# fengpeng-yue/speech-to-speech-translation

Measured on AMD Instinct MI355X. Metric: mel-frames/sec (fwd+bwd+opt) on Fisher-shaped fbank80->mel80, higher is better.
Workload: dtype bf16; 1 GPU; s2st_transformer base 12enc/6dec d512 nfps4 + aux ASR/ST(1x64) + CTC, recipe dropouts, max-tokens=20000 Fisher-shaped batches, update-freq 1; parallelism=dp1

## Files before the change

include/s2st_hip.h:

```cpp
#ifndef S2ST_HIP_H
#define S2ST_HIP_H
#include <stdint.h>
#ifdef __cplusplus
extern "C" {
#endif

#define S2ST_OK 0
#define S2ST_ERR_LAUNCH (-1)
#define S2ST_ERR_SHAPE (-2)
#define S2ST_ERR_WORKSPACE (-3)
#define S2ST_ERR_ARG (-4)
#define S2ST_ERR_COMM (-5)

typedef struct { int64_t ld; int64_t bs; int32_t per; int32_t _pad; } s2st_split;

typedef struct {
  const void* p;
  int32_t kmajor;
  int32_t dtype;
  s2st_split sp;
  int64_t zo, zi;
} s2st_gemm_operand;

#define S2ST_F32 0
// ... 212 lines not shown
int s2st_engine_create(const s2st_model_config* cfg, s2st_engine** out);
void s2st_engine_destroy(s2st_engine* e);
int32_t s2st_engine_num_params(const s2st_engine* e);
int s2st_engine_param_info(const s2st_engine* e, int32_t i, s2st_param_info* out);
int64_t s2st_engine_param_floats(const s2st_engine* e);
int64_t s2st_engine_buffer_floats(const s2st_engine* e);
int s2st_engine_bind(s2st_engine* e, float* params, float* grads, float* buffers);
int s2st_engine_bind_bf16(s2st_engine* e, uint16_t* params_bf16);
int s2st_engine_bf16_is_fresh(s2st_engine* e);
int64_t s2st_engine_stall_report(s2st_engine* e, int32_t verbose);
#define S2ST_SITE_LINEAR 1
#define S2ST_SITE_ATTN 2
#define S2ST_SITE_ROWS 3
#define S2ST_SITE_NORM 4
typedef struct s2st_dropout_site {
  uint64_t seed;
  int32_t kind;
  int32_t ordinal;
  float p;
  int32_t reserved;
  int64_t dims[5];
  char ctx[24];
} s2st_dropout_site;
int s2st_engine_allow_side_stream(s2st_engine* e, int32_t allow);
int s2st_engine_site_log(s2st_engine* e, int32_t on);
int32_t s2st_engine_site_log_get(const s2st_engine* e, s2st_dropout_site* out, int32_t cap);
int s2st_engine_bind_bf16_transposed(s2st_engine* e, uint16_t* params_bf16_t);
int64_t s2st_engine_workspace_floats(s2st_engine* e, const s2st_batch* geometry);
int s2st_engine_forward(s2st_engine* e, const s2st_batch* b, const s2st_outputs* out,
                        float* workspace, int64_t workspace_floats, void* stream);
int s2st_engine_backward(s2st_engine* e, float gscale, int32_t segment, void* stream);
int32_t s2st_engine_num_segments(const s2st_engine* e);
void* s2st_engine_side_stream(const s2st_engine* e);
int s2st_engine_segment_range(const s2st_engine* e, int32_t i, int64_t* lo, int64_t* hi);
int s2st_engine_adam_overlapped(s2st_engine* e, float* exp_avg, float* exp_avg_sq, const float* sumsq_parts, int32_t n_parts, float gmul, const float* gmul_dev, float max_norm, float lr, float beta1, float beta2, float eps, float wd, int32_t step, float* gnorm_out, int32_t* skipped, int32_t write_bf16, int32_t n_chunks, void* stream);
int s2st_engine_wait_optimizer(s2st_engine* e, void* stream);

int64_t s2st_engine_decode_state_floats(const s2st_engine* e, int32_t B, int32_t E, int32_t max_steps);
int s2st_engine_decode_begin(s2st_engine* e, const s2st_batch* b, const s2st_outputs* out, float* state,
                             int64_t state_floats, int32_t max_steps, float* workspace,
                             int64_t workspace_floats, void* stream);
int s2st_engine_decode_row_map(s2st_engine* e, const int32_t* row_map);
int s2st_engine_decode_step(s2st_engine* e, int32_t step, const float* prev, const int32_t* pos,
                            const int32_t* self_klen ,
                            uint64_t seed, float* feat_out, float* eos_prob, float* attn_out, float* workspace,
                            int64_t workspace_floats, void* stream);

typedef struct {
  int32_t* step;
  uint64_t* seeds;
  float* cur_feat;
  float* cur_eos;
  float* cur_attn;
  float* pe_cur;
} s2st_decode_replay;
int32_t s2st_engine_decode_replay_supported(const s2st_engine* e);
int s2st_engine_decode_replay_begin(s2st_engine* e, const s2st_decode_replay* r, uint64_t seed0, void* stream);
int s2st_engine_decode_step_replay(s2st_engine* e, const s2st_decode_replay* r, const int32_t* self_klen, float* workspace,
                                   int64_t workspace_floats, void* stream);
int s2st_engine_decode_replay_commit(s2st_engine* e, const s2st_decode_replay* r, uint64_t seed0, float thr, int32_t max_iter,
                                     int32_t* finished, int32_t* out_lens, int32_t* klen_next, int32_t* n_done,
                                     float* feat_all, float* eos_all, float* attn_all, void* stream);
int s2st_engine_postnet_eval(s2st_engine* e, const float* feat, int32_t B, int32_t D, float* post_out,
                             float* workspace, int64_t workspace_floats, void* stream);

int s2st_argmax_dim1_f32(const float* x, int64_t* idx, int32_t B, int32_t E, int32_t D, void* stream);
// ... 105 lines not shown
```

speech-to-speech-translation_amd/csrc/engine.cpp:

```cpp
#include <cmath>
#include <cstdio>
#include <cstdlib>
#include <cstring>
#include <functional>
#include <string>
#include <vector>

#include "s2st_ops.h"
#include <hip/hip_ext.h>

namespace {

struct PInfo {
  std::string name;
  long off, numel;
  int ndim;
  int shape[4];
  int is_buffer;
};

struct Ten {
  float* d = nullptr;
  float* g = nullptr;
  bf16raw* h = nullptr;
// ... 17 lines not shown
struct LinP { long w, b; int N, K; };
struct LNP { long g, b; int C; };
struct AttnP { long kvq_w, kvq_b, out_w, out_b; };
struct XAttnP { long kv_w, kv_b, q_w, q_b, out_w, out_b; };
struct EncLayerP { AttnP sa; LNP ln1; LinP fc1, fc2; LNP ln2; };
struct DecLayerP { AttnP sa; LNP ln1; XAttnP xa; LNP ln2; LinP fc1, fc2; LNP ln3; };
struct ConvP { long w, b; int O, I, Kw; };
struct BNP { long g, b, rm, rv; int C; };
struct AuxP {
  long embed; int V, in_dim, d, layers, out_dim;
  long proj_in;
  std::vector<DecLayerP> L;
  LNP ln; bool has_ln;
  long proj_out;
  long out_proj;
};

}

struct s2st_engine {
  s2st_model_config c;
  std::vector<PInfo> infos;
  long n_params = 0, n_buffers = 0;
  float *P = nullptr, *G = nullptr, *BUF = nullptr;
  hipStream_t side_ = nullptr;
  hipEvent_t ev_fork_ = nullptr, ev_join_ = nullptr, ev_taps_ = nullptr;
  bool overlap_aux = true;
  bool hoist_kv = true;
  hipEvent_t ev_kv_ = nullptr;
  bool kv_wait_ = false;
  hipEvent_t ev_auxb_ = nullptr;
  size_t aux_wait_idx = 0, aux_lo_idx = 0, aux_hi_idx = 0;
  bool aux_bwd_on_side = false;
  bool side_used = false;
  float* skws_side = nullptr;
  bool side_allowed = false;
  bool side_tried = false;
  void ensure_side() {
    if (side_ || side_tried || !side_allowed) return;
    side_tried = true;
    int pr_least = 0, pr_greatest = 0;
    if (hipDeviceGetStreamPriorityRange(&pr_least, &pr_greatest) != hipSuccess) pr_least = 0;
    if (hipStreamCreateWithPriority(&side_, hipStreamNonBlocking, pr_least) != hipSuccess) side_ = nullptr;
    if (side_ && hipEventCreateWithFlags(&ev_kv_, hipEventDisableTiming) != hipSuccess) ev_kv_ = nullptr;
    if (side_ && (hipEventCreateWithFlags(&ev_fork_, hipEventDisableTiming) != hipSuccess ||
                  hipEventCreateWithFlags(&ev_join_, hipEventDisableTiming) != hipSuccess ||
                  hipEventCreateWithFlags(&ev_taps_, hipEventDisableTiming) != hipSuccess ||
                  hipEventCreateWithFlags(&ev_auxb_, hipEventDisableTiming) != hipSuccess)) {
      hipStreamDestroy(side_);
      side_ = nullptr;
    }
  }
  hipStream_t fork_side() {
    if (!side_) { sync_chains(); return st_; }
    hipEventRecord(ev_fork_, st_);
    hipStreamWaitEvent(side_, ev_fork_, 0);
    if (forked_) {
      hipEventRecord(ev_cside_, chain1_);
      hipStreamWaitEvent(side_, ev_cside_, 0);
    }
    side_used = true;
    return side_;
  }
  struct Stall { const char* what; hipEvent_t a, b; };
  std::vector<Stall> stalls;
  bool stall_trace = false;
  void wait_traced(hipStream_t st, hipEvent_t ev, const char* what) {
    if (!stall_trace) { hipStreamWaitEvent(st, ev, 0); return; }
    Stall s{what, nullptr, nullptr};
    hipEventCreate(&s.a);
    hipEventCreate(&s.b);
    hipEventRecord(s.a, st);
    hipStreamWaitEvent(st, ev, 0);
    hipEventRecord(s.b, st);
    stalls.push_back(s);
  }
  void join_side() {
    sync_chains();
    if (!side_ || !side_used) return;
    hipEventRecord(ev_join_, side_);
    wait_traced(st_, ev_join_, "join_side");
    side_used = false;
  }

// ... 211 lines not shown
  e->use_skinny = !(s2st_env_on("S2ST_NO_SKINNY"));
  e->use_ln_fuse = !(s2st_env_on("S2ST_NO_LN_FUSE"));
  e->attn_gfuse_mode = s2st_env_int("S2ST_ATTN_GFUSE", 1);
  e->use_attn_gfuse = e->attn_gfuse_mode != 0;
  e->ln_bwd_split = s2st_env_on("S2ST_LN_BWD_SPLIT");
  e->ordered_sums = !(s2st_env_int("S2ST_ORDERED_BIAS_SUMS", 1) == 0);
  e->build_params();
  (void)hipGetLastError();
  if (!cfg->precise && (s2st_gemm_bf16_preload(nullptr) != 0 || s2st_flash_attn_preload(nullptr) != 0)) { delete e; return S2ST_ERR_LAUNCH; }
  e->side_allowed = !cfg->precise && !(s2st_env_on("S2ST_NO_SIDE_STREAM"));
  e->overlap_aux = !(s2st_env_on("S2ST_NO_AUX_OVERLAP"));
  if (!cfg->precise && s2st_env_int("S2ST_CHAINS", 1) == 2) {
    if (hipStreamCreateWithFlags(&e->chain1_, hipStreamNonBlocking) == hipSuccess &&
        hipEventCreateWithFlags(&e->ev_cfork_, hipEventDisableTiming) == hipSuccess &&
        hipEventCreateWithFlags(&e->ev_cjoin_, hipEventDisableTiming) == hipSuccess &&
        hipEventCreateWithFlags(&e->ev_cside_, hipEventDisableTiming) == hipSuccess)
      e->nchains = 2;
    else { delete e; return S2ST_ERR_LAUNCH; }
  }
  *out = e;
  return 0;
}

void s2st_engine_destroy(s2st_engine* e) {
  if (!e) return;
  if (e->side_) {
    hipStreamSynchronize(e->side_);
    hipStreamDestroy(e->side_);
    hipEventDestroy(e->ev_fork_);
    hipEventDestroy(e->ev_join_);
    if (e->ev_taps_) hipEventDestroy(e->ev_taps_);
    if (e->ev_auxb_) hipEventDestroy(e->ev_auxb_);
    if (e->ev_kv_) hipEventDestroy(e->ev_kv_);
    for (hipEvent_t ev : e->adam_ev) hipEventDestroy(ev);
  }
  if (e->chain1_) {
    hipStreamSynchronize(e->chain1_);
    hipStreamDestroy(e->chain1_);
    if (e->ev_cfork_) hipEventDestroy(e->ev_cfork_);
    if (e->ev_cjoin_) hipEventDestroy(e->ev_cjoin_);
    if (e->ev_cside_) hipEventDestroy(e->ev_cside_);
  }
  e->reset_call();
  delete e;
}

int32_t s2st_engine_num_params(const s2st_engine* e) { return (int32_t)e->infos.size(); }

int s2st_engine_param_info(const s2st_engine* e, int32_t i, s2st_param_info* out) {
  if (i < 0 || i >= (int)e->infos.size()) return S2ST_ERR_ARG;
  const PInfo& p = e->infos[i];
  memset(out, 0, sizeof(*out));
  strncpy(out->name, p.name.c_str(), sizeof(out->name) - 1);
  out->offset = p.off;
  out->numel = p.numel;
  out->ndim = p.ndim;
  for (int k = 0; k < 4; ++k) out->shape[k] = p.shape[k];
  out->is_buffer = p.is_buffer;
  return 0;
}

int64_t s2st_engine_param_floats(const s2st_engine* e) { return e->n_params; }
int64_t s2st_engine_buffer_floats(const s2st_engine* e) { return e->n_buffers; }

int s2st_engine_bind(s2st_engine* e, float* params, float* grads, float* buffers) {
  e->P = params;
// ... 78 lines not shown
}

int s2st_engine_backward(s2st_engine* e, float gscale, int32_t segment, void* stream) {
  if (!e->G) return S2ST_ERR_ARG;
  e->st_ = (hipStream_t)stream;
  e->gscale = gscale;
  if (segment < 0) {
    for (int s = 0; s < e->n_segments(); ++s) {
      int rc = e->backward_segment(s);
      if (rc) return rc;
    }
    return 0;
  }
  return e->backward_segment(segment);
}

int s2st_engine_adam_overlapped(s2st_engine* e, float* exp_avg, float* exp_avg_sq, const float* sumsq_parts, int32_t n_parts,
                                float gmul, const float* gmul_dev, float max_norm, float lr, float beta1, float beta2, float eps,
                                float wd, int32_t step, float* gnorm_out, int32_t* skipped, int32_t write_bf16, int32_t n_chunks,
                                void* stream) {
  if (!e || !exp_avg || !exp_avg_sq || !sumsq_parts || n_parts <= 0) return S2ST_ERR_ARG;
  return e->adam_overlapped(exp_avg, exp_avg_sq, sumsq_parts, n_parts, gmul, gmul_dev, max_norm, lr, beta1, beta2, eps, wd, step,
                            gnorm_out, skipped, write_bf16, n_chunks, (hipStream_t)stream);
}

int s2st_engine_wait_optimizer(s2st_engine* e, void* stream) {
  if (!e) return S2ST_ERR_ARG;
  e->adam_wait_all((hipStream_t)stream);
  return 0;
}

int32_t s2st_engine_num_segments(const s2st_engine* e) { return e->n_segments(); }

void* s2st_engine_side_stream(const s2st_engine* e) {
  const_cast<s2st_engine*>(e)->ensure_side();
  return (void*)e->side_;
}

int s2st_engine_segment_range(const s2st_engine* e, int32_t i, int64_t* lo, int64_t* hi) {
  int ns = e->n_segments();
  if (i < 0 || i >= ns) return S2ST_ERR_ARG;
  *lo = e->marks[ns - i - 1].param_off;
  *hi = e->marks[ns - i].param_off;
  return 0;
}

int64_t s2st_engine_decode_state_floats(const s2st_engine* e, int32_t B, int32_t E, int32_t max_steps) {
  const long Cd = e->c.dec_dim, L = e->c.dec_layers;
  return L * 2 * B * (long)max_steps * Cd + L * (long)B * E * 2 * Cd + 64 + ((long)max_steps + 2) * Cd + L * (long)B * E * Cd + 8;
}

int s2st_engine_decode_begin(s2st_engine* e, const s2st_batch* b, const s2st_outputs* out, float* state,
                             int64_t state_floats, int32_t max_steps, float* workspace, int64_t workspace_floats,
                             void* stream) {
  if (!e->P || !e->BUF || !state || !b || !out) return S2ST_ERR_ARG;
  if (state_floats < s2st_engine_decode_state_floats(e, b->B, b->E, max_steps)) return S2ST_ERR_WORKSPACE;
  e->dec_row_map = nullptr;
  e->begin_call(workspace, workspace_floats, stream);
  e->bt = *b;
  e->bt.training = 0;
  e->bt.tgt = nullptr;
  e->outs = *out;
  e->stop_after_encoder = true;
  int rc = e->forward();
  e->stop_after_encoder = false;
  if (rc) return rc;
  e->dec_st.base = state;
  e->dec_st.B = b->B; e->dec_st.E = b->E; e->dec_st.maxT = max_steps;
  e->dec_st.enc_lens = b->enc_lens;
  e->dec_st.pe_dec = b->pe_dec;
  {
    const long Cd = e->c.dec_dim, L = e->c.dec_layers;
    e->dec_st.pe_alpha = state + L * 2 * b->B * (long)max_steps * Cd + L * (long)b->B * b->E * 2 * Cd + 64;
    e->touch(e->pos_alpha + 1);
    if (e->live())
      e->chk(s2st_scale_rows(b->pe_dec, e->P + e->pos_alpha, e->dec_st.pe_alpha, ((long)max_steps + 2) * Cd, e->st_));
  }
  for (int l = 0; l < e->c.dec_layers; ++l) {
    const XAttnP& xa = e->dec[l].xa;
    e->linear(e->enc_out_keep, xa.kv_w, xa.kv_b, 2 * e->c.dec_dim, e->c.enc_dim, 0, 0.f, nullptr, e->dec_crossKV(l));
  }
  return e->end_call(0);
}

int s2st_engine_decode_row_map(s2st_engine* e, const int32_t* row_map) {
  if (!e) return S2ST_ERR_ARG;
  e->dec_row_map = row_map;
  return S2ST_OK;
}

int s2st_engine_decode_step(s2st_engine* e, int32_t step, const float* prev, const int32_t* pos,
                            const int32_t* self_klen, uint64_t seed, float* feat_out, float* eos_prob,
                            float* attn_out, float* workspace, int64_t workspace_floats, void* stream) {
  if (!e->P || !prev || !pos || !feat_out || !eos_prob) return S2ST_ERR_ARG;
  e->begin_call(workspace, workspace_floats, stream);
  if (int rc = e->params_ready(false, false)) return rc;
// ... 217 lines not shown
```

speech-to-speech-translation_amd/csrc/engine_ops.h:

```cpp
  Ten* linear(Ten* x, long w, long b, int N, int K, int act = 0, float drop_p = 0.f,
              Ten* resid = nullptr, float* ext_out = nullptr, bool only_h = false, const float* resid_row = nullptr) {
    const int M = x->rows;
    const bool fm = fast();
    const bool skinny = fm && !bt.training && use_skinny && M <= S2ST_SKINNY_MAX_ROWS && K % 32 == 0 && x->d && x->cols == K &&
                        (act == 0 || act == 1 || act == 3);
    only_h = only_h && fast() && use_only_h && N % 8 == 0 && !ext_out && !resid && !skinny;
    Ten* y = newT(M, N, ext_out, !only_h);
    touch(w + (long)N * K);
    if (b >= 0) touch(b + N);
    const uint64_t sd = drop_p > 0.f ? next_seed(S2ST_SITE_LINEAR, drop_p, M, N) : 0;
    if (skinny) {
      const uint64_t* seed_ptr = nullptr;
      if (replay_ && drop_p > 0.f) {
        if (site < 1 || site > 8) { if (!err) err = S2ST_ERR_SHAPE; return y; }
        seed_ptr = replay_->seeds + (site - 1);
      }
      if (live())
        chk(s2st_gemm_skinny(x->d, K, PH + w, K, y->d, N, b >= 0 ? P + b : nullptr, act, drop_p, sd,
                             resid ? resid->d : resid_row, resid ? N : 0, M, N, K, st_, nullptr, nullptr, 1e-5f, seed_ptr,
                             drop_p > 0.f ? dec_row_map : nullptr));
      return y;
    }
    if (replay_ && drop_p > 0.f && !err) err = S2ST_ERR_SHAPE;
    const bf16raw* xh = fm ? half_of(x) : nullptr;
// ... 380 lines not shown
      bool aq, ak, av;
      float* gq = gradbuf(io2.qt, aq);
      float* gk = gradbuf(io2.kt, ak);
      float* gv = gradbuf(io2.vt, av);
      (void)aq; (void)ak; (void)av;
      float* dp = alloc((long)B * H * T * ld);
      bf16raw* dsh = fm ? alloc_h((long)B * H * T * ld) : nullptr;
      const bf16raw* doh = fm ? ghalf_of(o) : nullptr;
      if (!live()) return;
      const View Vdo{o->g, doh};
      bgemm(Vdo, 1, C, (long)T * C, Vv, 1, io2.ldv, (long)S * io2.ldv, dp, ld, pzo, pzi, dh, dh, T, S, dh, 1.f);
      bgemm(View{pd, pdh}, 0, ld, pzo, Vdo, 0, C, (long)T * C, gv + io2.voff, io2.ldv, (long)S * io2.ldv, dh, pzi,
            dh, S, dh, T, 1.f);
      chk(s2st_softmax_bwd(p, dp, dp, B, H, T, S, ld, drop_p, sd, st_, dsh));
      bgemm(View{dp, dsh}, 1, ld, pzo, Vk, 0, io2.ldk, (long)S * io2.ldk, gq + io2.qoff, io2.ldq,
            (long)T * io2.ldq, dh, pzi, dh, T, dh, S, scaling);
      bgemm(View{dp, dsh}, 0, ld, pzo, Vq, 0, io2.ldq, (long)T * io2.ldq, gk + io2.koff, io2.ldk,
            (long)S * io2.ldk, dh, pzi, dh, S, dh, T, scaling);
    });
    return o;
  }

  Ten* self_attn_block(Ten* x, const AttnP& a, int B, int T, int H, const int* klen, int causal,
                       Ten* resid) {
    const int C = x->cols;
    Ten* kvq = linear(x, a.kvq_w, a.kvq_b, 3 * C, C, 0, 0.f, nullptr, nullptr, true);
    AttnIO io{kvq, 2 * C, 3 * C, kvq, 0, 3 * C, kvq, C, 3 * C};
    Ten* o = attention(io, B, T, T, H, C / H, klen, causal, bt.training ? c.attn_dropout : 0.f, nullptr);
    return linear(o, a.out_w, a.out_b, C, C, 0, bt.training ? c.dropout : 0.f, resid);
  }
  Ten* cross_kv(Ten* encx, const XAttnP& a, int C) {
    return linear(encx, a.kv_w, a.kv_b, 2 * C, encx->cols, 0, 0.f, nullptr, nullptr, true);
  }
  Ten* cross_attn_block(Ten* x, Ten* encx, const XAttnP& a, int B, int T, int S, int H,
                        const int* klen, Ten* resid, float* attn_mean_out, Ten* kv_pre = nullptr) {
    const int C = x->cols;
    Ten* q = linear(x, a.q_w, a.q_b, C, C, 0, 0.f, nullptr, nullptr, true);
    Ten* kv = kv_pre ? kv_pre : cross_kv(encx, a, C);
    if (kv_pre && kv_wait_) {
      wait_traced(st_, ev_kv_, "cross-attention K|V projections");
      chains_wait(ev_kv_);
      kv_wait_ = false;
    }
    AttnIO io{q, 0, C, kv, 0, 2 * C, kv, C, 2 * C};
    Ten* o = attention(io, B, T, S, H, C / H, klen, 0, bt.training ? c.attn_dropout : 0.f, attn_mean_out);
    return linear(o, a.out_w, a.out_b, C, C, 0, bt.training ? c.dropout : 0.f, resid);
  }
  Ten* ffn_block(Ten* x, const LinP& fc1, const LinP& fc2, Ten* resid) {
    Ten* h = linear(x, fc1.w, fc1.b, fc1.N, fc1.K, ffn_act, bt.training ? c.act_dropout : 0.f, nullptr, nullptr,
                    ffn_act == 1 || is_hubert);
    return linear(h, fc2.w, fc2.b, fc2.N, fc2.K, 0, bt.training ? c.dropout : 0.f, resid);
  }
  Ten* enc_layer(Ten* x, const EncLayerP& l, int B, int T) {
    const int H = c.enc_heads;
    if (c.enc_pre_ln) {
      x = self_attn_block(layernorm(x, l.ln1, nullptr, true), l.sa, B, T, H, bt.enc_lens, 0, x);
      return ffn_block(layernorm(x, l.ln2, nullptr, true), l.fc1, l.fc2, x);
    }
    x = layernorm(self_attn_block(x, l.sa, B, T, H, bt.enc_lens, 0, x), l.ln1);
    return layernorm(ffn_block(x, l.fc1, l.fc2, x), l.ln2);
  }
  Ten* dec_layer(Ten* x, Ten* encx, const DecLayerP& l, int B, int T, int S, int H, bool pre_ln,
                 const int* self_klen, float* attn_mean_out, Ten* kv_pre = nullptr) {
    if (pre_ln) {
      x = self_attn_block(layernorm(x, l.ln1, nullptr, true), l.sa, B, T, H, self_klen, 1, x);
      x = cross_attn_block(layernorm(x, l.ln2, nullptr, true), encx, l.xa, B, T, S, H, bt.enc_lens, x, attn_mean_out, kv_pre);
      return ffn_block(layernorm(x, l.ln3, nullptr, true), l.fc1, l.fc2, x);
    }
    x = layernorm(self_attn_block(x, l.sa, B, T, H, self_klen, 1, x), l.ln1);
    x = layernorm(cross_attn_block(x, encx, l.xa, B, T, S, H, bt.enc_lens, x, attn_mean_out, kv_pre), l.ln2);
    return layernorm(ffn_block(x, l.fc1, l.fc2, x), l.ln3);
  }

  struct ConvIn { float* xh; Ten* src; int Tin; const bf16raw* xhh; };
  struct ConvW { float *wf, *wd, *dwf; const bf16raw *wfh, *wdh; };
  Ten* conv(const ConvIn& in, const ConvP& p, int B, int stride, const ConvW& cw) {
    float *wf = cw.wf, *wd = cw.wd, *dwf = cw.dwf;
    const bf16raw *wfh = cw.wfh, *wdh = cw.wdh;
    const bool fm = fast();
    const int pad = p.Kw / 2;
    const int Tin = in.Tin, Tout = (Tin + 2 * pad - p.Kw) / stride + 1;
    const int Th = Tin + 2 * pad;
    Ten* z = newT(B * Tout, p.O);
    touch(p.w + (long)p.O * p.I * p.Kw);
    touch(p.b + p.O);
    if (live()) {
      GemmArgs g{};
      g.A = fm ? gemm_rowmajor(in.xhh, (long)stride * p.I) : gemm_rowmajor(in.xh, (long)stride * p.I);
      g.A.sp.per = Tout; g.A.sp.bs = (long)Th * p.I;
      g.B = fm ? gemm_rowmajor(wfh, (long)p.Kw * p.I) : gemm_rowmajor(wf, (long)p.Kw * p.I);
      g.C = gemm_out(z->d, p.O);
      g.ep = gemm_epi_default();
      g.ep.bias = P + p.b;
      g.M = B * Tout; g.N = p.O; g.K = p.Kw * p.I; g.batch = 1; g.zdiv = 1; g.precise = c.precise;
      chk(s2st_gemm(g, st_));
    }
    ConvP pp = p;
    ConvIn in2 = in;
    tape.push_back([=]() {
      if (!z->g) return;
      const int M = B * Tout;
      const bf16raw* dzh = fm ? ghalf_of(z) : nullptr;
      float* cpart = ordered_sums ? alloc(s2st_colsum_scratch_floats(M, pp.O)) : nullptr;
// ... 132 lines not shown
```

speech-to-speech-translation_amd/csrc/engine_step.h:

```cpp
  bool use_streamk = s2st_env_on("S2ST_GEMM_STREAMK");
  void reset_call() {
    pending_wgrad.clear();
    pending_lnfold = s2st_lnfold_table{};
    s2st_gemm_streamk_unbind_all();
    for (Ten* t : tens) delete t;
    tens.clear();
    tape.clear();
    tape_aware.clear();
    forked_ = false;
    in_region_ = false;
    marks.clear();
    ws_top = 0;
    ws_peak = 0;
    oom = false;
    err = 0;
    site = 0;
    site_log.clear();
    site_ctx[0] = 0;
    param_watermark = 0;
    next_segment = 0;
    skws = nullptr; skws_n = 0; skws_side = nullptr;
  }
  void begin_call(float* workspace, long workspace_floats, void* stream) {
    reset_call();
    dry = false;
    ws = workspace;
    ws_cap = workspace_floats;
    st_ = (hipStream_t)stream;
  }
  int params_ready(bool chunked = false, bool refresh = true) {
    if (dry) return 0;
    const bool fm = fast();
    if (fm && !PH) return S2ST_ERR_ARG;
    if (adam_pending && !(chunked && fm && ph_fresh)) adam_wait_all(st_);
    if (fm && refresh) {
      if (!ph_fresh) chk(s2st_cast_bf16_rows(P, n_params, PH, n_params, 1, (int)n_params, st_));
      ph_fresh = false;
    }
    return err;
  }
  int end_call(int rc) {
    tape.clear();
    return rc ? rc : err;
  }

  int forward() {
    const int B = bt.B, S = bt.S, D = bt.D, C = c.enc_dim, Cd = c.dec_dim;
    const int pad = c.conv_k / 2;
    const int T1 = c.text_input ? S : (S + 2 * pad - c.conv_k) / 2 + 1;
    const int T2 = c.text_input ? S : (T1 + 2 * pad - c.conv_k) / 2 + 1;
    if (T2 != bt.E) return S2ST_ERR_SHAPE;
    if (c.text_input && (!bt.src_txt || bt.Ls != S)) return S2ST_ERR_ARG;
    const int E = T2;
    const bool tr = bt.training != 0;
    const bool with_loss = bt.tgt != nullptr;
    seed = bt.seed;
    if (tr) ensure_side();
    main_ = st_;
    forked_ = false;
    in_region_ = false;
    const bool two_chains = nchains == 2 && chain1_ && tr && fast();

    const float *pe_enc = bt.pe_enc, *pe_dec = bt.pe_dec, *pe_asr = bt.pe_asr, *pe_st = bt.pe_st;
    const bool fm = fast();
    if (int rc = params_ready(true)) return rc;
    pht_valid = false;
    if (fm && tr && PHT && live()) {
      hipStream_t ts = side_ ? fork_side() : st_;
      if (wt_tables.empty()) build_wt_tables();
      for (const s2st_transpose_table& tb : wt_tables) chk(s2st_transpose_bf16_batched(PH, PHT, tb, ts));
      pht_valid = true;
    }
    skws_n = fm ? (long)16 << 20 : 0;
    skws = fm ? alloc(skws_n) : nullptr;
    skws_side = fm && side_allowed ? alloc(skws_n) : skws;
    skws_c1 = fm && chain1_ && nchains == 2 ? alloc(skws_n) : skws;
    if (fm && tr && use_streamk) {
      float* sk0 = alloc(S2ST_STREAMK_SCRATCH_FLOATS);
      float* sk1 = side_allowed ? alloc(S2ST_STREAMK_SCRATCH_FLOATS) : nullptr;
      if (live()) {
        hipMemsetAsync(sk0, 0, 4096, st_);
        s2st_gemm_streamk_bind(st_, sk0, S2ST_STREAMK_SCRATCH_FLOATS);
        if (sk1 && side_) {
          hipMemsetAsync(sk1, 0, 4096, st_);
          s2st_gemm_streamk_bind(side_, sk1, S2ST_STREAMK_SCRATCH_FLOATS);
        }
      }
    }
    typedef ConvW ConvScratch;
    auto conv_scratch = [&](const ConvP& p, bool need_wd) { return make_conv_scratch(p, need_wd, tr); };
    ConvScratch cs0{}, cs1{};
    std::vector<ConvScratch> cst;
    if (c.text_input) {
      for (auto& pc : enc_conv) cst.push_back(conv_scratch(pc, true));
    } else {
      cs0 = conv_scratch(sub[0], false);
      cs1 = conv_scratch(sub[1], true);
    }
    std::vector<ConvScratch> csp;
    {
      const bool post_on_side = fm && side_ && ev_taps_ && ev_kv_ && live() && hoist_kv && !stop_after_encoder &&
                                c.dec_layers > 0;
      hipStream_t main_st = st_;
      if (post_on_side) st_ = fork_side();
      for (auto& pc : post_conv) csp.push_back(conv_scratch(pc, true));
      st_ = main_st;
    }

    mark();
    Ten* x = nullptr;
    if (c.text_input) {
      Ten* emb = newT(B * E, C);
      touch(enc_embed + (long)c.src_vocab * C);
      if (live()) chk(s2st_embed_fwd((const long*)bt.src_txt, P + enc_embed, emb->d, B * E, C, 1.f, st_));
      const long eoff = enc_embed;
      tape.push_back([=]() {
        if (!emb->g) return;
        if (live()) chk(s2st_embed_bwd((const long*)bt.src_txt, emb->g, G + eoff, B * E, C, 1.f, 1, st_, ordered_sums ? c.src_vocab : 0));
      });
      set_ctx("enc.prenet");
      Ten* pn = text_prenet(emb, B, E, tr, cst);
      Ten* pj = linear(pn, enc_prenet_proj.w, enc_prenet_proj.b, C, C);
      set_ctx("enc.pe");
      x = add_pe(pj, bt.enc_pos, pe_enc, 1.f, enc_pos_alpha, tr ? c.dropout : 0.f);
    } else {
    float* xh0 = fm ? nullptr : alloc((long)B * (S + 2 * pad) * c.in_dim, true);
    if (live() && !fm) {
      Split xs{(long)c.in_dim, 0, 0, 0};
      Split ys{(long)c.in_dim, (long)(S + 2 * pad) * c.in_dim, S, 0};
      chk(s2st_copy_rows(bt.src, xs, xh0 + (long)pad * c.in_dim, ys, B * S, c.in_dim, st_));
    }
    const bf16raw* xh0h = fm ? cast_halo(bt.src, B, S, pad, c.in_dim, true) : nullptr;
    Ten* z1 = conv(ConvIn{xh0, nullptr, S, xh0h}, sub[0], B, 2, cs0);
    const int C1 = c.conv_channels / 2;
    float* g1h = alloc((long)B * (T1 + 2 * pad) * C1, !fm);
    Ten* g1 = glu_to(z1, g1h + (long)pad * C1, Split{(long)C1, (long)(T1 + 2 * pad) * C1, T1, 0}, C1);
    const bf16raw* g1hh = fm ? cast_halo(g1h, B, T1, pad, C1) : nullptr;
    Ten* z2 = conv(ConvIn{g1h, g1, T1, g1hh}, sub[1], B, 2, cs1);
// ... 32 lines not shown
        if (!c.spk_frozen && live())
          chk(s2st_speaker_cols_bwd(cat->g, (const long*)bt.speaker, B, E, C + Sd, C, Sd, c.n_speakers, G + soff, st_));
        if (xin->needs_grad) {
          bool acc;
          float* dx = gradbuf(xin, acc);
          if (live()) chk(s2st_split_cols(cat->g, C + Sd, dx, C, B * E, C, acc ? 1 : 0, st_));
        }
      });
      enc_out = linear(cat, enc_spk_proj.w, enc_spk_proj.b, C, C + Sd, 0, 0.f, nullptr, outs.enc_out);
    } else if (!has_enc_ln && outs.enc_out && live())
      hipMemcpyAsync(outs.enc_out, x->d, sizeof(float) * (size_t)x->n(), hipMemcpyDeviceToDevice, st_);
    if (!c.has_asr && tap_asr && outs.tap0 && live())
      hipMemcpyAsync(outs.tap0, tap_asr->d, sizeof(float) * (size_t)tap_asr->n(), hipMemcpyDeviceToDevice, st_);
    if (c.has_asr && tap_asr) tap_asr = layernorm(tap_asr, asr_norm, outs.tap0);
    if (c.has_st && tap_st) tap_st = layernorm(tap_st, st_norm, outs.tap1);
    const bool aux_on_side = side_ && ev_taps_ && live() && overlap_aux && !(c.text_input && c.has_ctc);
    const bool kv_on_side = side_ && ev_taps_ && ev_kv_ && live() && hoist_kv && !stop_after_encoder;
    if (aux_on_side || kv_on_side) hipEventRecord(ev_taps_, st_);
    aux_wait_idx = tape.size();
    mark();
    if (stop_after_encoder) {
      enc_out_keep = enc_out;
      return err;
    }
    if (c.s2t_mode) return forward_s2t(enc_out, with_loss);
    std::vector<Ten*> xkv(c.dec_layers, nullptr);
    if (hoist_kv) {
      hipStream_t main_st = st_;
      if (kv_on_side) {
        hipStreamWaitEvent(side_, ev_taps_, 0);
        st_ = side_;
        side_used = true;
      }
      for (int i = 0; i < c.dec_layers; ++i) xkv[i] = cross_kv(enc_out, dec[i].xa, Cd);
      if (kv_on_side) {
        hipEventRecord(ev_kv_, side_);
        st_ = main_st;
        kv_wait_ = true;
      }
      mark();
    }
    Ten* prev = newT(B * D, c.out_dim, const_cast<float*>(bt.prev));
    prev->needs_grad = false;
    if (dec_spk >= 0 && bt.speaker) {
      Ten* pv = newT(B * D, c.out_dim);
      touch_spk(dec_spk + (long)c.n_speakers * c.out_dim);
      if (live()) {
        hipMemcpyAsync(pv->d, bt.prev, sizeof(float) * (size_t)pv->n(), hipMemcpyDeviceToDevice, st_);
        chk(s2st_speaker_set_rows(spk_tab(dec_spk), (const long*)bt.speaker, pv->d, B, D, c.out_dim, st_));
      }
      pv->needs_grad = tr && !c.spk_frozen;
      const long doff = dec_spk;
      tape.push_back([=]() {
        if (!pv->g || c.spk_frozen) return;
        if (live())
          chk(s2st_speaker_bwd(pv->g, (const long*)bt.speaker, B, D, 1, c.out_dim, c.n_speakers, 0.f, 0, G + doff, st_));
      });
      prev = pv;
    }
    Ten* h = prev;
    set_ctx("dec.prenet");
    for (int i = 0; i < c.prenet_layers; ++i)
      h = linear(h, prenet[i].w, prenet[i].b, prenet[i].N, prenet[i].K, 1, c.prenet_dropout);
    h = linear(h, prenet.back().w, prenet.back().b, Cd, c.prenet_dim);
    set_ctx("dec.pe");
    Ten* y = add_pe(h, bt.dec_pos, pe_dec, 1.f, pos_alpha, tr ? c.dropout : 0.f);
    mark();
    in_region_ = two_chains;
    float* attn_out = nullptr;
    Ten* tap_dec_t = nullptr;
    for (int i = 0; i < c.dec_layers; ++i) {
      float* am = (i == c.dec_layers - 1 && bt.want_attn) ? outs.attn : nullptr;
      set_ctx("dec.L%d", i);
      y = dec_layer(y, enc_out, dec[i], B, D, E, c.dec_heads, c.dec_pre_ln != 0, bt.tgt_lens, am, xkv[i]);
      if (c.has_ctc_tgt && i == c.tap_dec) tap_dec_t = y;
      if (i % 2 == 1) mark();
    }
    (void)attn_out;
    if (has_dec_ln) y = layernorm(y, dec_ln);
    Ten* feat = linear(y, feat_proj.w, feat_proj.b, c.out_dim, Cd, 0, 0.f, nullptr, outs.feat);
    Ten* eos = linear(y, eos_proj.w, eos_proj.b, 1, Cd, 0, 0.f, nullptr, outs.eos);
    in_region_ = false;
    if (live()) sync_chains();
    set_ctx("post");
    Ten* post = postnet(feat, B, D, tr, csp, outs.post_feat);
    set_ctx("");
    Ten* ctc_tgt_logits = nullptr;
    float *ctc_tgt_per = nullptr, *ctc_tgt_dl = nullptr;
    if (c.has_ctc_tgt && tap_dec_t) {
      ctc_tgt_logits = linear(tap_dec_t, ctc_proj_tgt.w, ctc_proj_tgt.b, c.tgt_vocab, Cd);
      if (with_loss) {
        ctc_tgt_per = alloc(B);
        float* lp = alloc((long)B * D * c.tgt_vocab);
        float* wsd = alloc(s2st_ctc_workspace_floats(B, D, bt.Lt));
        ctc_tgt_dl = tr ? alloc(ctc_tgt_logits->n()) : nullptr;
        if (live())
          chk(s2st_ctc(ctc_tgt_logits->d, (const long*)bt.tgt_txt, bt.Lt, bt.tgt_lens, bt.tgt_txt_lens, B, D, c.tgt_vocab,
                       lp, ctc_tgt_per, ctc_tgt_dl, ctc_tgt_dl ? c.ctc_tgt_weight / B : 0.f, wsd, st_));
      }
    }
    mark();
    hipStream_t main_st = st_;
    aux_lo_idx = tape.size();
    if (aux_on_side) {
      hipStreamWaitEvent(side_, ev_taps_, 0);
      st_ = side_;
      side_used = true;
    }
    Ten* ctc_logits = nullptr;
    if (c.has_ctc && tap_asr && !c.text_input) ctc_logits = linear(tap_asr, ctc_proj.w, ctc_proj.b, c.src_vocab, C);
    const bool t2s_ctc = c.text_input && c.has_ctc;
// ... 113 lines not shown
        chk(s2st_loss_finalize(stats, nullptr, B, 1.f, 1.f, 0.f, 0.f, 0.f, 0.f, 1.f, 0.f, c.label_smoothing, c.tgt_vocab,
                               c.tgt_vocab, 1.f, 1.f, st_, nullptr, 0.f, ordered_sums ? &lp : nullptr));
      }
      tape.push_back([=]() {
        bool a;
        float* dl = gradbuf(logits, a);
        if (live())
          chk(s2st_ls_ce(logits->d, (const long*)bt.src_txt, B * bt.Ls, c.tgt_vocab, 1, c.label_smoothing, nullptr, dl,
                         gscale, st_));
      });
    }
    if (adam_pending && live()) adam_wait_all(st_);
    join_side();
    mark();
    return err;
  }

  int n_segments() const { return marks.empty() ? 0 : (int)marks.size() - 1; }

  int backward_segment(int seg) {
    int ns = n_segments();
    if (seg < 0 || seg >= ns) return S2ST_ERR_ARG;
    if (seg == 0) join_side();
    size_t hi = marks[ns - seg].tape_idx, lo = marks[ns - seg - 1].tape_idx;
    hipStream_t main_st = st_;
    main_ = st_;
    in_region_ = false;
    for (size_t i = hi; i-- > lo;) {
      if (aux_bwd_on_side && live()) {
        if (i + 1 == aux_hi_idx && st_ == main_st) { flush_wgrad(); flush_lnfold(); st_ = fork_side(); }
        if (i + 1 == aux_lo_idx && st_ != main_st) { flush_wgrad(); flush_lnfold(); hipEventRecord(ev_auxb_, st_); st_ = main_st; }
        if (i + 1 == aux_wait_idx) wait_traced(main_st, ev_auxb_, "aux decoders' backward (tap gradients)");
      }
      if (live() && !(i < tape_aware.size() && tape_aware[i])) sync_chains();
      tape[i]();
      if (err) break;
    }
    flush_wgrad();
    flush_lnfold();
    if (st_ != main_st) { hipEventRecord(ev_auxb_, st_); st_ = main_st; }
    if (live()) sync_chains();
    if (seg == ns - 1) join_side();
    return err;
  }
```

speech-to-speech-translation_amd/runtime/engine.py:

```python
from __future__ import annotations

import ctypes as C
import math
import os
from typing import Callable, Dict, List, Optional, Tuple

import torch

from . import binding as bd

PAD = 1


class ModelConfig(C.Structure):
    _fields_ = [(n, C.c_int32) for n in (
        "enc_layers", "dec_layers", "enc_dim", "dec_dim", "enc_ffn", "dec_ffn", "enc_heads",
        "dec_heads", "enc_pre_ln", "dec_pre_ln", "in_dim", "conv_channels", "conv_k", "out_dim",
        "prenet_layers", "prenet_dim", "postnet_layers", "postnet_dim", "postnet_k", "tap_asr",
        "tap_st", "has_asr", "has_st", "has_ctc", "asr_layers", "asr_dim", "st_layers", "st_dim",
        "src_vocab", "tgt_vocab", "no_scale_embedding", "precise", "tap_dec", "has_ctc_tgt", "text_input", "enc_conv_layers", "enc_conv_k",
        "n_speakers", "spk_frozen", "spk_dim")] + [(n, C.c_float) for n in (
        "dropout", "attn_dropout", "act_dropout", "prenet_dropout", "postnet_dropout", "ctc_weight",
        "asr_weight", "st_weight", "w_l1", "w_mse", "w_eos", "bce_pos_weight", "label_smoothing", "ctc_tgt_weight", "enc_dropout")] + \
        [("s2t_mode", C.c_int32)]
# ... 650 lines not shown
    def site_log(self, on: bool = True):
        bd.check(self.lib.s2st_engine_site_log(self.h, 1 if on else 0), "s2st_engine_site_log")

    def dropout_sites(self) -> Dict[str, "DropoutSite"]:
        f = self.lib.s2st_engine_site_log_get
        n = int(f(self.h, None, 0))
        recs = (DropoutSite * max(n, 1))()
        f(self.h, C.cast(recs, C.c_void_p), n)
        out = {}
        for r in recs[:n]:
            name = f"{r.ctx.decode()}/{SITE_KIND[r.kind]}{r.ordinal}"
            assert name not in out, name
            out[name] = r
        return out

    def dropout_keep_mask(self, site: "DropoutSite") -> torch.Tensor:
        d = [int(v) for v in site.dims]
        shape = (d[0], d[1], d[2], d[4]) if site.kind == 2 else (d[0], d[1])
        n = 1
        for v in shape:
            n *= v
        ones = torch.ones(n, dtype=torch.float32, device=self.device)
        y = torch.empty_like(ones)
        bd.call("s2st_dropout_f32", ones, y, n, 1.0, float(site.p), int(site.seed), 0)
        keep = (y != 0).float()
        return keep.view(*shape)

    def side_stream(self):
        if bd.is_emulator() or not torch.cuda.is_available():
            return None
        p = self.lib.s2st_engine_side_stream(self.h)
        return torch.cuda.ExternalStream(p) if p else None

    def num_segments(self) -> int:
        return int(self.lib.s2st_engine_num_segments(self.h))

    def segment_range(self, i: int) -> Tuple[int, int]:
        lo, hi = C.c_int64(), C.c_int64()
        bd.check(self.lib.s2st_engine_segment_range(self.h, i, C.byref(lo), C.byref(hi)), "segment_range")
        return int(lo.value), int(hi.value)

    def backward(self, gscale: float = 1.0,
                 on_segment: Optional[Callable[[int, int, int], None]] = None):
        if on_segment is None:
            bd.check(self.lib.s2st_engine_backward(self.h, gscale, -1, bd.stream_ptr()), "s2st_engine_backward")
            return
        for i in range(self.num_segments()):
            bd.check(self.lib.s2st_engine_backward(self.h, gscale, i, bd.stream_ptr()), "s2st_engine_backward")
            lo, hi = self.segment_range(i)
            if hi > lo:
                on_segment(i, lo, hi)

    def adam_overlapped(self, exp_avg, exp_avg_sq, sumsq_parts, n_parts, gmul, gmul_dev, max_norm, lr, beta1, beta2, eps, wd,
                        step, gnorm_out, skipped, write_bf16: bool, n_chunks: int = 8):
        f = self.lib.s2st_engine_adam_overlapped
        for t in (exp_avg, exp_avg_sq, sumsq_parts, gnorm_out, skipped):
            bd.require_device(t)
        bd.check(f(self.h, exp_avg.data_ptr(), exp_avg_sq.data_ptr(), sumsq_parts.data_ptr(), int(n_parts), float(gmul),
                   bd.ptr(gmul_dev), float(max_norm), float(lr), float(beta1), float(beta2), float(eps), float(wd), int(step),
                   gnorm_out.data_ptr(), skipped.data_ptr(), 1 if write_bf16 else 0, int(n_chunks), bd.stream_ptr()),
                 "s2st_engine_adam_overlapped")

    def wait_optimizer(self):
        bd.check(self.lib.s2st_engine_wait_optimizer(self.h, bd.stream_ptr()), "s2st_engine_wait_optimizer")

    def zero_grad(self):
# ... 2 lines not shown
```

Before: 1.435 million mel-frames/s.

## Overlap decoder front with encoder and run decoder-tail backward on side stream

```diff
diff --git a/include/s2st_hip.h b/include/s2st_hip.h
--- a/include/s2st_hip.h
+++ b/include/s2st_hip.h
@@ -268,6 +268,7 @@
 int s2st_engine_backward(s2st_engine* e, float gscale, int32_t segment, void* stream);
 int32_t s2st_engine_num_segments(const s2st_engine* e);
 void* s2st_engine_side_stream(const s2st_engine* e);
+int32_t s2st_engine_dec_overlap_active(const s2st_engine* e);
 int s2st_engine_segment_range(const s2st_engine* e, int32_t i, int64_t* lo, int64_t* hi);
 int s2st_engine_adam_overlapped(s2st_engine* e, float* exp_avg, float* exp_avg_sq, const float* sumsq_parts, int32_t n_parts, float gmul, const float* gmul_dev, float max_norm, float lr, float beta1, float beta2, float eps, float wd, int32_t step, float* gnorm_out, int32_t* skipped, int32_t write_bf16, int32_t n_chunks, void* stream);
 int s2st_engine_wait_optimizer(s2st_engine* e, void* stream);
diff --git a/speech-to-speech-translation_amd/csrc/engine.cpp b/speech-to-speech-translation_amd/csrc/engine.cpp
--- a/speech-to-speech-translation_amd/csrc/engine.cpp
+++ b/speech-to-speech-translation_amd/csrc/engine.cpp
@@ -73,6 +73,13 @@
   hipEvent_t ev_auxb_ = nullptr;
   size_t aux_wait_idx = 0, aux_lo_idx = 0, aux_hi_idx = 0;
   bool aux_bwd_on_side = false;
+  int dec_overlap = 3;
+  hipEvent_t ev_head_ = nullptr;
+  bool side_events_ = false;
+  size_t tail_lo_idx = 0, tail_hi_idx = 0;
+  bool tail_bwd_on_side = false, tail_side_ = false;
+  bool dec_early_active = false;
+  size_t xattn0_idx = 0;
   bool side_used = false;
   float* skws_side = nullptr;
   bool side_allowed = false;
@@ -83,7 +90,10 @@
     int pr_least = 0, pr_greatest = 0;
     if (hipDeviceGetStreamPriorityRange(&pr_least, &pr_greatest) != hipSuccess) pr_least = 0;
     if (hipStreamCreateWithPriority(&side_, hipStreamNonBlocking, pr_least) != hipSuccess) side_ = nullptr;
-    if (side_ && hipEventCreateWithFlags(&ev_kv_, hipEventDisableTiming) != hipSuccess) ev_kv_ = nullptr;
+    if (!side_ && !chain1_ && hipStreamCreateWithFlags(&side_, hipStreamNonBlocking) != hipSuccess) side_ = nullptr;
+    bool ev_ok = side_ != nullptr;
+    if (side_ && hipEventCreateWithFlags(&ev_kv_, hipEventDisableTiming) != hipSuccess) { ev_kv_ = nullptr; ev_ok = false; }
+    if (side_ && hipEventCreateWithFlags(&ev_head_, hipEventDisableTiming) != hipSuccess) { ev_head_ = nullptr; ev_ok = false; }
     if (side_ && (hipEventCreateWithFlags(&ev_fork_, hipEventDisableTiming) != hipSuccess ||
                   hipEventCreateWithFlags(&ev_join_, hipEventDisableTiming) != hipSuccess ||
                   hipEventCreateWithFlags(&ev_taps_, hipEventDisableTiming) != hipSuccess ||
@@ -91,6 +101,7 @@
       hipStreamDestroy(side_);
       side_ = nullptr;
     }
+    side_events_ = side_ && ev_ok;
   }
   hipStream_t fork_side() {
     if (!side_) { sync_chains(); return st_; }
@@ -368,6 +379,7 @@
     if (e->ev_taps_) hipEventDestroy(e->ev_taps_);
     if (e->ev_auxb_) hipEventDestroy(e->ev_auxb_);
     if (e->ev_kv_) hipEventDestroy(e->ev_kv_);
+    if (e->ev_head_) hipEventDestroy(e->ev_head_);
     for (hipEvent_t ev : e->adam_ev) hipEventDestroy(ev);
   }
   if (e->chain1_) {
@@ -512,6 +524,10 @@
 
 int32_t s2st_engine_num_segments(const s2st_engine* e) { return e->n_segments(); }
 
+int32_t s2st_engine_dec_overlap_active(const s2st_engine* e) {
+  return e ? (e->dec_early_active ? 1 : 0) | (e->tail_bwd_on_side ? 2 : 0) : 0;
+}
+
 void* s2st_engine_side_stream(const s2st_engine* e) {
   const_cast<s2st_engine*>(e)->ensure_side();
   return (void*)e->side_;
@@ -542,6 +558,7 @@
   e->bt.tgt = nullptr;
   e->outs = *out;
   e->stop_after_encoder = true;
+  e->adam_wait_all((hipStream_t)stream);
   int rc = e->forward();
   e->stop_after_encoder = false;
   if (rc) return rc;
diff --git a/speech-to-speech-translation_amd/csrc/engine_ops.h b/speech-to-speech-translation_amd/csrc/engine_ops.h
--- a/speech-to-speech-translation_amd/csrc/engine_ops.h
+++ b/speech-to-speech-translation_amd/csrc/engine_ops.h
@@ -436,10 +436,9 @@
   Ten* cross_kv(Ten* encx, const XAttnP& a, int C) {
     return linear(encx, a.kv_w, a.kv_b, 2 * C, encx->cols, 0, 0.f, nullptr, nullptr, true);
   }
-  Ten* cross_attn_block(Ten* x, Ten* encx, const XAttnP& a, int B, int T, int S, int H,
+  Ten* cross_attn_block(Ten* q, Ten* encx, const XAttnP& a, int B, int T, int S, int H,
                         const int* klen, Ten* resid, float* attn_mean_out, Ten* kv_pre = nullptr) {
-    const int C = x->cols;
-    Ten* q = linear(x, a.q_w, a.q_b, C, C, 0, 0.f, nullptr, nullptr, true);
+    const int C = q->cols;
     Ten* kv = kv_pre ? kv_pre : cross_kv(encx, a, C);
     if (kv_pre && kv_wait_) {
       wait_traced(st_, ev_kv_, "cross-attention K|V projections");
@@ -448,6 +447,7 @@
     }
     AttnIO io{q, 0, C, kv, 0, 2 * C, kv, C, 2 * C};
     Ten* o = attention(io, B, T, S, H, C / H, klen, 0, bt.training ? c.attn_dropout : 0.f, attn_mean_out);
+    if (kv_pre && !xattn0_idx) xattn0_idx = tape.size() - 1;
     return linear(o, a.out_w, a.out_b, C, C, 0, bt.training ? c.dropout : 0.f, resid);
   }
   Ten* ffn_block(Ten* x, const LinP& fc1, const LinP& fc2, Ten* resid) {
@@ -464,15 +464,26 @@
     x = layernorm(self_attn_block(x, l.sa, B, T, H, bt.enc_lens, 0, x), l.ln1);
     return layernorm(ffn_block(x, l.fc1, l.fc2, x), l.ln2);
   }
+  struct DecHead { Ten* x = nullptr; Ten* q = nullptr; };
+  DecHead dec_head(Ten* x, const DecLayerP& l, int B, int T, int H, bool pre_ln, const int* self_klen) {
+    DecHead h;
+    Ten* xn;
+    if (pre_ln) {
+      h.x = self_attn_block(layernorm(x, l.ln1, nullptr, true), l.sa, B, T, H, self_klen, 1, x);
+      xn = layernorm(h.x, l.ln2, nullptr, true);
+    } else {
+      h.x = xn = layernorm(self_attn_block(x, l.sa, B, T, H, self_klen, 1, x), l.ln1);
+    }
+    const int C = xn->cols;
+    h.q = linear(xn, l.xa.q_w, l.xa.q_b, C, C, 0, 0.f, nullptr, nullptr, true);
+    return h;
+  }
   Ten* dec_layer(Ten* x, Ten* encx, const DecLayerP& l, int B, int T, int S, int H, bool pre_ln,
-                 const int* self_klen, float* attn_mean_out, Ten* kv_pre = nullptr) {
-    if (pre_ln) {
-      x = self_attn_block(layernorm(x, l.ln1, nullptr, true), l.sa, B, T, H, self_klen, 1, x);
-      x = cross_attn_block(layernorm(x, l.ln2, nullptr, true), encx, l.xa, B, T, S, H, bt.enc_lens, x, attn_mean_out, kv_pre);
-      return ffn_block(layernorm(x, l.ln3, nullptr, true), l.fc1, l.fc2, x);
-    }
-    x = layernorm(self_attn_block(x, l.sa, B, T, H, self_klen, 1, x), l.ln1);
-    x = layernorm(cross_attn_block(x, encx, l.xa, B, T, S, H, bt.enc_lens, x, attn_mean_out, kv_pre), l.ln2);
+                 const int* self_klen, float* attn_mean_out, Ten* kv_pre = nullptr, const DecHead* head = nullptr) {
+    const DecHead h = head ? *head : dec_head(x, l, B, T, H, pre_ln, self_klen);
+    x = cross_attn_block(h.q, encx, l.xa, B, T, S, H, bt.enc_lens, h.x, attn_mean_out, kv_pre);
+    if (pre_ln) return ffn_block(layernorm(x, l.ln3, nullptr, true), l.fc1, l.fc2, x);
+    x = layernorm(x, l.ln2);
     return layernorm(ffn_block(x, l.fc1, l.fc2, x), l.ln3);
   }
 
diff --git a/speech-to-speech-translation_amd/csrc/engine_step.h b/speech-to-speech-translation_amd/csrc/engine_step.h
--- a/speech-to-speech-translation_amd/csrc/engine_step.h
+++ b/speech-to-speech-translation_amd/csrc/engine_step.h
@@ -16,6 +16,8 @@
     err = 0;
     site = 0;
     site_log.clear();
+    xattn0_idx = 0;
+    tail_bwd_on_side = tail_side_ = dec_early_active = false;
     site_ctx[0] = 0;
     param_watermark = 0;
     next_segment = 0;
@@ -60,6 +62,7 @@
     forked_ = false;
     in_region_ = false;
     const bool two_chains = nchains == 2 && chain1_ && tr && fast();
+    dec_overlap = s2st_env_int("S2ST_DEC_OVERLAP", 3);
 
     const float *pe_enc = bt.pe_enc, *pe_dec = bt.pe_dec, *pe_asr = bt.pe_asr, *pe_st = bt.pe_st;
     const bool fm = fast();
@@ -104,6 +107,58 @@
       hipStream_t main_st = st_;
       if (post_on_side) st_ = fork_side();
       for (auto& pc : post_conv) csp.push_back(conv_scratch(pc, true));
+      st_ = main_st;
+    }
+
+    const bool kv_side_ok = side_ && side_events_ && hoist_kv && !stop_after_encoder;
+    const bool dec_early = tr && fm && (dec_overlap & 1) && kv_side_ok && !two_chains && !c.text_input && !c.s2t_mode &&
+                           c.dec_layers > 0 && bt.prev && !(dec_spk >= 0 && bt.speaker);
+    struct {
+      std::vector<std::function<void()>> tape;
+      std::vector<s2st_dropout_site> log;
+      size_t n_front = 0;
+      long wm_front = 0, wm_head = 0;
+      uint64_t site_first = 0, site_lo = 0, site_hi = 0;
+      Ten* y = nullptr;
+      DecHead head;
+    } early;
+    auto dec_front = [&](Ten* prev) {
+      Ten* h = prev;
+      set_ctx("dec.prenet");
+      for (int i = 0; i < c.prenet_layers; ++i)
+        h = linear(h, prenet[i].w, prenet[i].b, prenet[i].N, prenet[i].K, 1, c.prenet_dropout);
+      h = linear(h, prenet.back().w, prenet.back().b, Cd, c.prenet_dim);
+      set_ctx("dec.pe");
+      return add_pe(h, bt.dec_pos, pe_dec, 1.f, pos_alpha, tr ? c.dropout : 0.f);
+    };
+    if (dec_early) {
+      const int n_enc_sites = (c.dropout > 0.f ? 1 : 0) +
+                              c.enc_layers * ((c.attn_dropout > 0.f ? 1 : 0) + (c.dropout > 0.f ? 2 : 0) + (c.act_dropout > 0.f ? 1 : 0));
+      hipStream_t main_st = st_;
+      const uint64_t site0 = site;
+      const long wm0 = param_watermark;
+      const size_t t0 = tape.size(), l0 = site_log.size();
+      early.site_first = site0;
+      early.site_lo = site = site0 + n_enc_sites;
+      if (live()) { st_ = fork_side(); dec_early_active = st_ == side_; }
+      Ten* prev = newT(B * D, c.out_dim, const_cast<float*>(bt.prev));
+      prev->needs_grad = false;
+      early.y = dec_front(prev);
+      early.n_front = tape.size() - t0;
+      early.wm_front = param_watermark;
+      set_ctx("dec.L%d", 0);
+      early.head = dec_head(early.y, dec[0], B, D, c.dec_heads, c.dec_pre_ln != 0, bt.tgt_lens);
+      early.wm_head = param_watermark;
+      early.site_hi = site;
+      early.tape.assign(std::make_move_iterator(tape.begin() + t0), std::make_move_iterator(tape.end()));
+      tape.resize(t0);
+      if (tape_aware.size() > t0) tape_aware.resize(t0);
+      early.log.assign(site_log.begin() + l0, site_log.end());
+      site_log.resize(l0);
+      site = site0;
+      param_watermark = wm0;
+      site_ctx[0] = 0;
+      if (live()) hipEventRecord(ev_head_, st_);
       st_ = main_st;
     }
 
@@ -202,14 +257,19 @@
         st_ = side_;
         side_used = true;
       }
-      for (int i = 0; i < c.dec_layers; ++i) xkv[i] = cross_kv(enc_out, dec[i].xa, Cd);
+      for (int i = 0; i < c.dec_layers; ++i) {
+        if (dec_early && i == 0) st_ = main_st;
+        xkv[i] = cross_kv(enc_out, dec[i].xa, Cd);
+        if (dec_early && i == 0 && kv_on_side) st_ = side_;
+      }
       if (kv_on_side) {
         hipEventRecord(ev_kv_, side_);
         st_ = main_st;
-        kv_wait_ = true;
+        kv_wait_ = !dec_early;
       }
       mark();
     }
+    tail_lo_idx = tape.size();
     Ten* prev = newT(B * D, c.out_dim, const_cast<float*>(bt.prev));
     prev->needs_grad = false;
     if (dec_spk >= 0 && bt.speaker) {
@@ -228,25 +288,46 @@
       });
       prev = pv;
     }
-    Ten* h = prev;
-    set_ctx("dec.prenet");
-    for (int i = 0; i < c.prenet_layers; ++i)
-      h = linear(h, prenet[i].w, prenet[i].b, prenet[i].N, prenet[i].K, 1, c.prenet_dropout);
-    h = linear(h, prenet.back().w, prenet.back().b, Cd, c.prenet_dim);
-    set_ctx("dec.pe");
-    Ten* y = add_pe(h, bt.dec_pos, pe_dec, 1.f, pos_alpha, tr ? c.dropout : 0.f);
-    mark();
+    Ten* y = nullptr;
+    auto file_early = [&](size_t lo, size_t hi, long wm) {
+      for (size_t k = lo; k < hi; ++k) tape.push_back(std::move(early.tape[k]));
+      tape_aware.resize(tape.size(), 0);
+      if (wm > param_watermark) param_watermark = wm;
+    };
+    if (dec_early) {
+      if (site != early.site_lo && !err) {
+        fprintf(stderr, "[s2st] S2ST_DEC_OVERLAP: %llu dropout sites reserved for the encoder, %llu drawn -- update n_enc_sites "
+                        "in forward() (engine_step.h)\n", (unsigned long long)(early.site_lo - early.site_first),
+                (unsigned long long)(site - early.site_first));
+        err = S2ST_ERR_SHAPE;
+      }
+      site = early.site_hi;
+      site_log.insert(site_log.end(), early.log.begin(), early.log.end());
+      y = early.y;
+      file_early(0, early.n_front, early.wm_front);
+      if (live()) wait_traced(st_, ev_head_, "decoder front issued ahead");
+    } else {
+      y = dec_front(prev);
+    }
+    mark();
+    if (dec_early) file_early(early.n_front, early.tape.size(), early.wm_head);
     in_region_ = two_chains;
     float* attn_out = nullptr;
     Ten* tap_dec_t = nullptr;
     for (int i = 0; i < c.dec_layers; ++i) {
       float* am = (i == c.dec_layers - 1 && bt.want_attn) ? outs.attn : nullptr;
       set_ctx("dec.L%d", i);
-      y = dec_layer(y, enc_out, dec[i], B, D, E, c.dec_heads, c.dec_pre_ln != 0, bt.tgt_lens, am, xkv[i]);
+      if (dec_early && kv_on_side && i == 1) kv_wait_ = true;
+      y = dec_layer(y, enc_out, dec[i], B, D, E, c.dec_heads, c.dec_pre_ln != 0, bt.tgt_lens, am, xkv[i],
+                    (dec_early && i == 0) ? &early.head : nullptr);
       if (c.has_ctc_tgt && i == c.tap_dec) tap_dec_t = y;
       if (i % 2 == 1) mark();
     }
     (void)attn_out;
+    if (tr && kv_side_ok && live() && !two_chains && (dec_overlap & 2) && xattn0_idx > tail_lo_idx) {
+      tail_hi_idx = xattn0_idx;
+      tail_bwd_on_side = true;
+    }
     if (has_dec_ln) y = layernorm(y, dec_ln);
     Ten* feat = linear(y, feat_proj.w, feat_proj.b, c.out_dim, Cd, 0, 0.f, nullptr, outs.feat);
     Ten* eos = linear(y, eos_proj.w, eos_proj.b, 1, Cd, 0, 0.f, nullptr, outs.eos);
@@ -426,13 +507,22 @@
         if (i + 1 == aux_lo_idx && st_ != main_st) { flush_wgrad(); flush_lnfold(); hipEventRecord(ev_auxb_, st_); st_ = main_st; }
         if (i + 1 == aux_wait_idx) wait_traced(main_st, ev_auxb_, "aux decoders' backward (tap gradients)");
       }
+      if (tail_bwd_on_side && live()) {
+        const bool in_tail = i >= tail_lo_idx && i < tail_hi_idx;
+        if (in_tail && st_ == main_st) { st_ = fork_side(); tail_side_ = true; }
+        if (!in_tail && tail_side_) { st_ = main_st; tail_side_ = false; }
+      }
       if (live() && !(i < tape_aware.size() && tape_aware[i])) sync_chains();
       tape[i]();
       if (err) break;
     }
     flush_wgrad();
     flush_lnfold();
-    if (st_ != main_st) { hipEventRecord(ev_auxb_, st_); st_ = main_st; }
+    if (st_ != main_st) {
+      if (!tail_side_) hipEventRecord(ev_auxb_, st_);
+      st_ = main_st;
+    }
+    tail_side_ = false;
     if (live()) sync_chains();
     if (seg == ns - 1) join_side();
     return err;
diff --git a/speech-to-speech-translation_amd/runtime/engine.py b/speech-to-speech-translation_amd/runtime/engine.py
--- a/speech-to-speech-translation_amd/runtime/engine.py
+++ b/speech-to-speech-translation_amd/runtime/engine.py
@@ -706,6 +706,9 @@
         p = self.lib.s2st_engine_side_stream(self.h)
         return torch.cuda.ExternalStream(p) if p else None
 
+    def dec_overlap_active(self) -> int:
+        return int(self.lib.s2st_engine_dec_overlap_active(self.h))
+
     def num_segments(self) -> int:
         return int(self.lib.s2st_engine_num_segments(self.h))
 
```

Result: faster. 1.458 million mel-frames/s, median of 6 (+1.6%).
